# JohnVithor/RL-Rust

Measured on AMD Instinct MI355X. Metric: env-steps/sec, FrozenLake-8x8 Q-learning, 2^20 envs, 1/2/4/8 GPUs, higher is better.
Workload: dtype f64 TD arithmetic; shared Q int64 fixed point 2^-40 (range proven, |Q| <= 2048, no clamp)

## Files before the change

### rl-rust_amd/csrc/rl_device.h

```cpp
#pragma once
#include <hip/hip_runtime.h>
#include <stdint.h>

#include "rl_kparams.h"
#include "rl_taxi.h"

#pragma clang fp contract(off)

namespace rlamd {

constexpr double MIN_POSITIVE = 2.2250738585072014e-308;

__device__ __forceinline__ uint32_t xor3(uint32_t a, uint32_t b, uint32_t c) {
    uint32_t r;
    asm("v_bitop3_b32 %0, %1, %2, %3 bitop3:0x96" : "=v"(r) : "v"(a), "v"(b), "v"(c));
    return r;
}
struct Rng {
    uint32_t s0, s1, s2, s3;
    __device__ __forceinline__ void advance() {
        const uint32_t t = s1 << 9;
        const uint32_t n1 = xor3(s1, s2, s0), n2 = xor3(s2, s0, t), n0 = xor3(s0, s3, s1), n3 = s3 ^ s1;
        s0 = n0; s1 = n1; s2 = n2;
        s3 = __builtin_rotateleft32(n3, 11);
// ... 251 lines not shown
        y = t - (e - x);
        y = add_exponent(y, k);
    } else {
        t = with_hi(0.0, (uint32_t)((0x3ff - k) << 20));
        y = x - (e + t);
        y += 1.0;
        y = add_exponent(y, k);
    }
    return y;
}

__device__ inline double rl_tanh(double x) {
    const double tiny = 1.0e-300;
    double t, z;
    const int32_t jx = (int32_t)hi_word(x);
    const int32_t ix = jx & 0x7fffffff;
    if (ix >= 0x7ff00000) {
        if (jx >= 0) return 1.0 / x + 1.0;
        return 1.0 / x - 1.0;
    }
    if (ix < 0x40360000) {
        if (ix < 0x3c800000) return x * (1.0 + x);
        if (ix >= 0x3ff00000) {
            t = rl_expm1(2.0 * __builtin_fabs(x));
            z = 1.0 - 2.0 / (t + 2.0);
        } else {
            t = rl_expm1(-2.0 * __builtin_fabs(x));
            z = -t / (t + 2.0);
        }
    } else {
        z = 1.0 - tiny;
    }
    return jx >= 0 ? z : -z;
}

__device__ __forceinline__ double max_rs(double a, double b) { return (a > b || b != b) ? a : b; }
__device__ __forceinline__ double min_rs(double a, double b) { return (a < b || b != b) ? a : b; }
__device__ __forceinline__ double sigmoid_(double v) { return 1.0 / (1.0 + rl_exp(-v)); }
template <int ACT>
__device__ __forceinline__ double act_t(double v) {
    if constexpr (ACT == RL_ACT_TANH) return rl_tanh(v);
    else if constexpr (ACT == RL_ACT_RELU) return max_rs(v, 0.0);
    else if constexpr (ACT == RL_ACT_LEAKY_RELU) return max_rs(v, 0.1 * v);
    else if constexpr (ACT == RL_ACT_RELU6) return min_rs(max_rs(v, 0.0), 6.0);
    else if constexpr (ACT == RL_ACT_LEAKY_RELU6) return __builtin_fmin(__builtin_fmax(v, 0.1 * v), 6.0);
    else if constexpr (ACT == RL_ACT_SIGMOID) return sigmoid_(v);
    else if constexpr (ACT == RL_ACT_SWISH) return v * sigmoid_(v);
    else if constexpr (ACT == RL_ACT_HARD_SWISH) return (v * min_rs(max_rs(v + 3.0, 0.0), 6.0)) / 6.0;
    else return v;
}
template <int ACT>
__device__ __forceinline__ double act_pt(double v) {
    if constexpr (ACT == RL_ACT_TANH) { const double t = rl_tanh(v); return 1.0 - t * t; }
    else if constexpr (ACT == RL_ACT_RELU) return v > 0.0 ? 1.0 : 0.0;
    else if constexpr (ACT == RL_ACT_LEAKY_RELU) return v > 0.0 ? 1.0 : 0.01;
    else if constexpr (ACT == RL_ACT_RELU6) return (v > 0.0 && v < 6.0) ? 1.0 : 0.0;
    else if constexpr (ACT == RL_ACT_LEAKY_RELU6) return (v > 0.0 && v < 6.0) ? 1.0 : 0.01;
    else if constexpr (ACT == RL_ACT_SIGMOID) { const double sg = sigmoid_(v); return sg * (1.0 - sg); }
    else if constexpr (ACT == RL_ACT_SWISH) { const double e = rl_exp(v); return (e * (v + e + 1.0)) / ((e + 1.0) * (e + 1.0)); }
    else if constexpr (ACT == RL_ACT_HARD_SWISH) return v > -3.0 ? (2.0 * v + 3.0) / 6.0 : 0.0;
    else return 1.0;
}
__device__ inline double act_f(int act, double v) {
    switch (act) {
    case RL_ACT_TANH: return act_t<RL_ACT_TANH>(v);
    case RL_ACT_RELU: return act_t<RL_ACT_RELU>(v);
    case RL_ACT_LEAKY_RELU: return act_t<RL_ACT_LEAKY_RELU>(v);
    case RL_ACT_RELU6: return act_t<RL_ACT_RELU6>(v);
    case RL_ACT_LEAKY_RELU6: return act_t<RL_ACT_LEAKY_RELU6>(v);
    case RL_ACT_SIGMOID: return act_t<RL_ACT_SIGMOID>(v);
    case RL_ACT_SWISH: return act_t<RL_ACT_SWISH>(v);
    case RL_ACT_HARD_SWISH: return act_t<RL_ACT_HARD_SWISH>(v);
    default: return v;
    }
}
__device__ inline double act_fp(int act, double v) {
    switch (act) {
    case RL_ACT_TANH: return act_pt<RL_ACT_TANH>(v);
    case RL_ACT_RELU: return act_pt<RL_ACT_RELU>(v);
    case RL_ACT_LEAKY_RELU: return act_pt<RL_ACT_LEAKY_RELU>(v);
    case RL_ACT_RELU6: return act_pt<RL_ACT_RELU6>(v);
    case RL_ACT_LEAKY_RELU6: return act_pt<RL_ACT_LEAKY_RELU6>(v);
    case RL_ACT_SIGMOID: return act_pt<RL_ACT_SIGMOID>(v);
    case RL_ACT_SWISH: return act_pt<RL_ACT_SWISH>(v);
    case RL_ACT_HARD_SWISH: return act_pt<RL_ACT_HARD_SWISH>(v);
    default: return 1.0;
    }
}

__device__ __forceinline__ double ucb_value(double q, double c, double lnt, double n) {
    return q + c * __builtin_sqrt(lnt / (n + MIN_POSITIVE));
}

template <int A>
__device__ __forceinline__ uint32_t ucb_known(const double (&v)[A], const uint64_t (&n)[A], double c, double lnt,
                                              double (&u)[A]) {
    const double b0 = c * __builtin_sqrt(lnt * 0x1p1022);
    const bool c_fin = __builtin_fabs(c) < 0x1p1020;
    uint32_t need = 0;
#pragma unroll
    for (int i = 0; i < A; ++i) {
        const bool z = n[i] == 0ull, nf = !__builtin_isfinite(v[i]) && c_fin;
        u[i] = z ? v[i] + b0 : (nf ? v[i] : 0.0);
        need |= (!z && !nf) ? (1u << i) : 0u;
    }
    return need;
}
template <int A>
__device__ __forceinline__ void ucb_fill(const double (&v)[A], const uint64_t (&n)[A], double c, double lnt,
                                         uint32_t need, double (&u)[A]) {
#pragma unroll
    for (int i = 0; i < A; ++i)
        if ((need >> i) & 1u) u[i] = ucb_value(v[i], c, lnt, (double)n[i]);
}

constexpr uint64_t QNAN_BITS = 0x7FF8000000000000ull;
__device__ __forceinline__ double as_f64(uint64_t u) { return __longlong_as_double((long long)u); }
__device__ __forceinline__ uint64_t f64_bits(double x) { return (uint64_t)__double_as_longlong(x); }
__device__ __forceinline__ double canon_nan(double x) { return x != x ? as_f64(QNAN_BITS) : x; }
__device__ __forceinline__ uint32_t f64_code(double x) {
    return ((uint32_t)((uint64_t)__double_as_longlong(x) >> 52)) & 0x7ffu;
}
__device__ __forceinline__ int fq_grid(uint32_t code) { return (int)(code > 1u ? code : 1u) - 1075; }
__device__ __forceinline__ uint32_t nf_flag(double x) { return x != x ? QF_NAN : (x > 0.0 ? QF_PINF : QF_NINF); }
__device__ __forceinline__ double nf_value(uint32_t f) {
    if ((f & QF_NAN) || ((f & QF_PINF) && (f & QF_NINF))) return as_f64(QNAN_BITS);
    return (f & QF_PINF) ? __builtin_inf() : -__builtin_inf();
}
__device__ __forceinline__ int64_t fq_raw(double d, int e) {
    return (int64_t)__builtin_rint(__builtin_ldexp(d, -e));
}
template <int A>
__device__ __forceinline__ uint32_t argmax_max_f64(const double (&v)[A], double &m) {
    m = v[0];
    uint32_t r = 0;
#pragma unroll
    for (int i = 1; i < A; ++i) {
        const bool gt = v[i] > m;
        m = gt ? v[i] : m;
        r = gt ? (uint32_t)i : r;
    }
    return r;
}

constexpr int64_t Q_RAW_MAX = (int64_t)1 << 51;

__device__ __forceinline__ int64_t rint_i64_small(double x) {
    const double y = x + 0x1.8p52;
    return (int64_t)((uint64_t)__double_as_longlong(y) - 0x4338000000000000ull);
}
__device__ __forceinline__ int64_t q_fix_inrange(double d) { return rint_i64_small(d * 0x1p40); }
__device__ __forceinline__ double q_val(int64_t raw) {
    return __longlong_as_double((long long)(0x40B8000000000000ull + (uint64_t)raw)) - 6144.0;
}
template <int A>
__device__ __forceinline__ uint32_t argmax_i64(const int64_t (&v)[A]) {
    int64_t m = v[0];
    uint32_t r = 0;
#pragma unroll
    for (int i = 1; i < A; ++i)
        if (v[i] > m) { m = v[i]; r = (uint32_t)i; }
    return r;
}
template <int A>
__device__ __forceinline__ int64_t max_i64(const int64_t (&v)[A]) {
    int64_t m = v[0];
#pragma unroll
    for (int i = 1; i < A; ++i) m = v[i] > m ? v[i] : m;
    return m;
}
template <class T>
__device__ __forceinline__ T opq(T x) {
    asm("" : "+v"(x));
    return x;
}
template <int A, class T>
__device__ __forceinline__ T pick(const T (&v)[A], uint32_t i) {
    T r = opq(v[0]);
#pragma unroll
    for (int j = 1; j < A; ++j) r = (i == (uint32_t)j) ? opq(v[j]) : r;
    return r;
}

template <int A>
__device__ __forceinline__ uint32_t argmax(const double (&v)[A]) {
    double m = v[0];
    uint32_t r = 0;
#pragma unroll
    for (int i = 1; i < A; ++i)
        if (v[i] > m) { m = v[i]; r = (uint32_t)i; }
    return r;
}
template <int A>
__device__ __forceinline__ double vmax(const double (&v)[A]) {
    double m = v[0];
#pragma unroll
    for (int i = 1; i < A; ++i)
        if (v[i] > m) m = v[i];
    return m;
}
__device__ __forceinline__ uint32_t cdf_search(const double *cdf, uint32_t n, double u) {
    uint32_t lo = 0, hi = n;
    while (lo < hi) {
        const uint32_t mid = (lo + hi) >> 1;
        if (cdf[mid] > u) hi = mid; else lo = mid + 1;
    }
    return lo < n ? lo : 0u;
}

struct EnvTables {
    const uint32_t *trans;
    const double *cdf;
    uint32_t n_start, max_steps;
    double th1, th2, th3, trunc_reward;
    int32_t fixed_start;
    int32_t slippery;
    uint32_t S;
};
template <bool AM, int A>
__device__ __forceinline__ uint32_t tidx(const EnvTables &t, uint32_t s, uint32_t a) {
    return AM ? a * t.S + s : s * (uint32_t)A + a;
}
__device__ __forceinline__ uint32_t start_state(const EnvTables &t, double u) {
    return t.fixed_start >= 0 ? (uint32_t)t.fixed_start : cdf_search(t.cdf, t.n_start, u);
}

__device__ __forceinline__ uint32_t start_list_search(const EnvTables &t, double u) {
    const uint32_t *cells = (const uint32_t *)(t.cdf + t.n_start);
    uint32_t c = 0;
    bool found = false;
    for (uint32_t j = 0; j < t.n_start; ++j) {
        const bool hit = !found && t.cdf[j] > u;
        c = hit ? cells[j] : c;
        found = found || hit;
    }
    return c;
}

template <int ENV> struct EnvDev;

template <bool EDITED, int SLIP, bool AM, bool MAPS = false>
__device__ __forceinline__ void fl_advance(bool doR, bool doS, uint32_t &pos, uint32_t &z, uint32_t w, Rng &r,
                                           const EnvTables &t, uint32_t &s2, double &rew, bool &term) {
    const bool trunc = doS && z >= t.max_steps;
    const bool st = doS && !trunc;
    uint32_t i = 0, s0 = 0;
    if constexpr (MAPS) {
        const bool slip = SLIP == 1 || (SLIP < 0 && t.slippery);
        const bool drawn = t.fixed_start < 0;
        s0 = drawn ? 0u : (uint32_t)t.fixed_start;
        if ((slip && st) || (drawn && doR)) {
            const double u = uniform01(r);
            const uint32_t iu = (t.th1 > u) ? 0u : (t.th2 > u) ? 1u : (t.th3 > u) ? 2u : 0u;
            i = (st && (w & (1u << 24))) ? iu : 0u;
            if (drawn) {
                const uint32_t c = start_list_search(t, u);
                s0 = doR ? c : 0u;
            }
        }
    } else if (SLIP == 1 || (SLIP < 0 && t.slippery)) {
        if (st) {
            const double u = uniform01(r);
            if (w & (1u << 24)) i = (t.th1 > u) ? 0u : (t.th2 > u) ? 1u : (t.th3 > u) ? 2u : 0u;
        }
    }
    const uint32_t o = (w >> (8 * i)) & 0xffu;
    const double r_bit = EDITED ? 10.0 : 1.0, r_else = EDITED ? -1.0 : 0.0;
    s2 = st ? (o & 63u) : ((EDITED && trunc) ? pos : (MAPS && doR ? s0 : 0u));
    rew = st ? ((o & 64u) ? r_bit : r_else) : ((EDITED && trunc) ? -1.0 : 0.0);
    term = trunc || (st && (o & 128u) != 0u);
    z = doR ? 0u : (st ? z + 1u : z);
    pos = s2;
}

template <> struct EnvDev<RL_ENV_FROZEN_LAKE> {
    static constexpr int A = 4;
    __device__ static __forceinline__ uint32_t reset(uint32_t &z, Rng &, const EnvTables &) {
        z = 0;
        return 0u;
    }
    template <int SLIP = -1, bool AM = false>
    __device__ static __forceinline__ void step(uint32_t &pos, uint32_t &z, uint32_t a, Rng &r,
                                                const EnvTables &t, uint32_t &s2, double &rew,
                                                bool &term) {
        if (z >= t.max_steps) { s2 = 0; rew = 0.0; term = true; return; }
        z += 1;
        const uint32_t w = t.trans[tidx<AM, 4>(t, pos, a)];
        uint32_t i = 0;
        if (SLIP == 1 || (SLIP < 0 && t.slippery)) {
            const double u = uniform01(r);
            if (w & (1u << 24)) i = (t.th1 > u) ? 0u : (t.th2 > u) ? 1u : (t.th3 > u) ? 2u : 0u;
        }
        const uint32_t o = (w >> (8 * i)) & 0xffu;
        s2 = o & 63u;
        rew = (o & 64u) ? 1.0 : 0.0;
        term = (o & 128u) != 0;
        pos = s2;
    }
};

template <> struct EnvDev<RL_ENV_FROZEN_LAKE_EDITED> {
    static constexpr int A = 4;
    __device__ static __forceinline__ uint32_t reset(uint32_t &z, Rng &, const EnvTables &) {
        z = 0;
        return 0u;
    }
// ... 263 lines not shown
```

### rl-rust_amd/csrc/rl_train_impl.h

```cpp
#pragma once
#include <type_traits>

#include "rl_device.h"
#include "rl_net.h"

namespace rlamd {

constexpr uint32_t POOL_ITEM_BYTES = 10u;
struct SmemLayout {
    uint32_t st, misc, q, sum, cnt, sfl, qf, n, nd, t, list, rcp, tr, cdf, lrec, trc, qd, rm, total;
    uint32_t trc_cap;
    uint32_t nrcp;
};
__host__ __device__ inline uint32_t align16(uint32_t x) { return (x + 15u) & ~15u; }

constexpr uint32_t BJ_LDS_STATES = 22u * 11u * 2u;
__host__ __device__ inline bool bj_compact(int env, int ucb) { return env == RL_ENV_BLACKJACK && !ucb; }
__host__ __device__ inline bool bj_nonterminal(uint32_t s) {
    const uint32_t p = s >> 6, d = (s >> 1) & 31u;
    return p <= 21u && d <= 10u;
}
__host__ __device__ inline uint32_t bj_row(uint32_t s) {
    const uint32_t p = s >> 6, r = s & 63u;
    return (p * 11u + (r >> 1)) * 2u + (r & 1u);
// ... 180 lines not shown
    e.pad[0] = e.pad[1] = e.pad[2] = 0;
    e.reward = L.epi_reward;
    p.elog[(uint64_t)(c % p.elog_cap) * p.L + lane] = e;
    p.elog_cnt[lane] = c + 1u;
}

__device__ __forceinline__ void write_record(const KParams &p, uint32_t k, uint64_t lane, uint32_t kind,
                                             uint32_t s, uint32_t a, uint32_t s2, uint32_t a2, double r,
                                             bool term, double td, uint32_t mode) {
    rl_step_record rec;
    rec.s = s;
    rec.s2 = s2;
    rec.a = (uint8_t)a;
    rec.a2 = (uint8_t)a2;
    rec.term = (uint8_t)term;
    rec.mode = (uint8_t)mode;
    rec.kind = (uint8_t)kind;
    rec.pad[0] = rec.pad[1] = rec.pad[2] = 0;
    rec.r = r;
    rec.td = td;
    p.rec[(uint64_t)k * p.L + lane] = rec;
}

template <int A>
__device__ __forceinline__ void trace_visit(const KParams &p, uint64_t lane, uint32_t s, uint32_t a,
                                            uint32_t &cnt) {
    const uint64_t Ls = p.L;
    uint32_t j = p.slot_of[(uint64_t)s * Ls + lane];
    if (j < cnt && p.tlist[(uint64_t)j * Ls + lane] == s) {
        double *e = &p.trace[((uint64_t)j * A + a) * Ls + lane];
        *e = *e + 1.0;
    } else {
        j = cnt++;
        p.tlist[(uint64_t)j * Ls + lane] = (uint16_t)s;
        p.slot_of[(uint64_t)s * Ls + lane] = (uint16_t)j;
#pragma unroll
        for (int b = 0; b < A; ++b) p.trace[((uint64_t)j * A + b) * Ls + lane] = (uint32_t)b == a ? 1.0 : 0.0;
    }
}

template <int A, class RowFn, class Fn>
__device__ __forceinline__ void trace_sweep(const KParams &p, uint64_t lane, uint32_t nv, RowFn &&row_fn, Fn &&fn) {
    constexpr uint32_t TC = 4;
    const uint64_t Ls = p.L;
    for (uint32_t j0 = 0; j0 < nv; j0 += TC) {
        uint32_t o[TC];
        double ev[TC][A];
#pragma unroll
        for (uint32_t c = 0; c < TC; ++c) {
            const bool in = j0 + c < nv;
            const uint32_t j = in ? j0 + c : j0;
            o[c] = p.tlist[(uint64_t)j * Ls + lane];
#pragma unroll
            for (int b = 0; b < A; ++b) ev[c][b] = p.trace[((uint64_t)j * A + b) * Ls + lane];
        }
#pragma unroll
        for (uint32_t c = 0; c < TC; ++c) {
            if (j0 + c < nv) {
                const uint32_t j = j0 + c;
                row_fn(o[c]);
#pragma unroll
                for (int b = 0; b < A; ++b) {
                    fn(o[c], (uint32_t)b, ev[c][b]);
                    p.trace[((uint64_t)j * A + b) * Ls + lane] = ev[c][b] * p.gl;
                }
            }
        }
    }
}

constexpr uint32_t SWEEP_U = 4;
__device__ __forceinline__ uint64_t pslot(const KParams &p, uint32_t j, uint64_t lane) {
    return lane * (uint64_t)(p.S * p.A) + j;
}
struct PairCache {
    uint16_t *TRI;
    double *TRE;
    uint32_t cap, nthr, tid;
    __device__ __forceinline__ uint32_t ixi_t(uint32_t j, uint32_t t) const { return j * (nthr + 2u) + t; }
    __device__ __forceinline__ uint32_t ixe_t(uint32_t j, uint32_t t) const { return j * (nthr + 1u) + t; }
    __device__ __forceinline__ uint32_t ixi(uint32_t j) const { return ixi_t(j, tid); }
    __device__ __forceinline__ uint32_t ixe(uint32_t j) const { return ixe_t(j, tid); }
};
template <int A>
__device__ __forceinline__ void pair_visit(const KParams &p, const PairCache &c, uint64_t lane, uint32_t s,
                                           uint32_t a, uint32_t &np) {
    const uint64_t Ls = p.L;
    const uint32_t id = s * (uint32_t)A + a, id0 = s * (uint32_t)A;
    const uint32_t nl = np < c.cap ? np : c.cap;
    uint32_t hit = 0xffffffffu;
    bool same_state = false;
    constexpr uint32_t TB = 8;
    for (uint32_t j0 = 0; j0 < nl; j0 += TB) {
        uint32_t w[TB];
#pragma unroll
        for (uint32_t k = 0; k < TB; ++k) w[k] = c.TRI[c.ixi(j0 + k < nl ? j0 + k : j0)] & 0x7fffu;
#pragma unroll
        for (uint32_t k = 0; k < TB; ++k) {
            if (j0 + k < nl) {
                if (w[k] == id) hit = j0 + k;
                if (w[k] - id0 < (uint32_t)A) same_state = true;
            }
        }
    }
    if (hit != 0xffffffffu) {
        c.TRE[c.ixe(hit)] += 1.0;
        return;
    }
    if (np > c.cap) {
        const uint32_t j = p.slot_of[(uint64_t)id * Ls + lane];
        if (j >= c.cap && j < np && (p.tlist[pslot(p, j, lane)] & 0x7fffu) == id) {
            double *e = &p.trace[pslot(p, j, lane)];
            *e = *e + 1.0;
            return;
        }
    }
    const uint32_t j = np++;
    if (j < c.cap) {
        c.TRI[c.ixi(j)] = (uint16_t)(id | (same_state ? 0u : 0x8000u));
        c.TRE[c.ixe(j)] = 1.0;
    } else {
        uint32_t *vw = &p.vbits[(uint64_t)(s >> 5) * Ls + lane];
        const uint32_t vb = *vw, bit = 1u << (s & 31u);
        const bool first = !same_state && (vb & bit) == 0u;
        if ((vb & bit) == 0u) *vw = vb | bit;
        p.tlist[pslot(p, j, lane)] = (uint16_t)(id | (first ? 0x8000u : 0u));
        p.slot_of[(uint64_t)id * Ls + lane] = (uint16_t)j;
        p.trace[pslot(p, j, lane)] = 1.0;
    }
}
__device__ __forceinline__ void pair_clear(const KParams &p, const PairCache &c, uint64_t lane, uint32_t np) {
    if (np <= c.cap) return;
    const uint32_t nw = (p.S + 31u) >> 5;
    for (uint32_t w = 0; w < nw; ++w) p.vbits[(uint64_t)w * p.L + lane] = 0u;
}
__device__ __forceinline__ void pair_cache_load(const KParams &p, const PairCache &c, uint64_t lane, uint32_t np) {
    const uint32_t nl = np < c.cap ? np : c.cap;
    for (uint32_t j = 0; j < nl; ++j) {
        c.TRI[c.ixi(j)] = p.tlist[pslot(p, j, lane)];
        c.TRE[c.ixe(j)] = p.trace[pslot(p, j, lane)];
    }
}
__device__ __forceinline__ void pair_cache_store(const KParams &p, const PairCache &c, uint64_t lane, uint32_t np) {
    const uint32_t nl = np < c.cap ? np : c.cap;
    for (uint32_t j = 0; j < nl; ++j) {
        p.tlist[pslot(p, j, lane)] = c.TRI[c.ixi(j)];
        p.trace[pslot(p, j, lane)] = c.TRE[c.ixe(j)];
    }
}

constexpr uint32_t QF_MASK = QF_NAN | QF_PINF | QF_NINF, QF_PENDING = 4u;
__device__ __forceinline__ uint32_t value_flags(double q) { return __builtin_isfinite(q) ? 0u : nf_flag(q); }

template <int AGENT, int POLICY, int SEL, int ALGO>
constexpr bool fix_possible() {
    return AGENT == RL_AGENT_ONE_STEP && POLICY == RL_POLICY_TABULAR &&
           !(SEL == RL_SEL_UCB && ALGO == RL_ALGO_EXPECTED_SARSA);
}

constexpr uint32_t CARVE_OWN = 0xffffffffu;
template <int ENV, int AGENT, int POLICY, int SEL, int ALGO, bool INSTR, bool FQ, int SLIP = -1, int SWEEP = -1,
          bool PACK = false, int RS = -1, int EPI = -1, bool POP = false>
__device__ __forceinline__ void train_shared_body(const KParams &p, unsigned long long *pop_row = nullptr,
                                                  uint32_t carve_n_start = CARVE_OWN) {
    using E = EnvDev<ENV>;
    constexpr int A = E::A;
    constexpr int P = POLICY == RL_POLICY_DOUBLE ? 2 : 1;
    constexpr bool UCB = SEL == RL_SEL_UCB;
    constexpr bool TRACES = AGENT == RL_AGENT_TRACES;
    constexpr bool SPEC = UCB && ALGO == RL_ALGO_EXPECTED_SARSA;
    static_assert(FQ || fix_possible<AGENT, POLICY, SEL, ALGO>(), "no range proof: f64 only");
    constexpr bool BJC = ENV == RL_ENV_BLACKJACK && !UCB;
    const uint32_t S = p.S, SA = S * (uint32_t)A, PSA = (uint32_t)P * SA;
    const uint32_t SL = BJC ? BJ_LDS_STATES : S, SAL = SL * (uint32_t)A, PSAL = (uint32_t)P * SAL;

    extern __shared__ __attribute__((aligned(16))) unsigned char smem[];
    const uint32_t tid = threadIdx.x, nthr = blockDim.x;
    constexpr bool PAIRS = TRACES && !SPEC;
    constexpr bool QSH = qsh_layout(FQ ? 1 : 0, UCB ? 1 : 0, P, ALGO);
    uint32_t carve_ns = p.n_start;
    if constexpr (POP) carve_ns = carve_n_start == CARVE_OWN ? p.n_start : carve_n_start;
    const SmemLayout lay = smem_layout(ENV, P, UCB ? (SPEC ? 2 : 1) : 0, TRACES ? (PAIRS ? 2 : 1) : 0, S, A, carve_ns,
                                       nthr, p.trc_kb, FQ ? 1 : 0, p.ucb_pack, QSH ? 1 : 0);
    unsigned long long *Q = (unsigned long long *)(smem + lay.q);
    double *QD = (double *)(smem + lay.qd);
    double2 *RM = (double2 *)(smem + lay.rm);
    unsigned long long *SUM = (unsigned long long *)(smem + lay.sum);
    uint32_t *CNT = (uint32_t *)(smem + lay.cnt);
    uint16_t *CNT16 = (uint16_t *)(smem + lay.cnt);
    uint32_t *W = (uint32_t *)(smem + lay.cnt);
    uint32_t *SFLW = (uint32_t *)(smem + (SPEC ? lay.qf : lay.sfl));
    uint8_t *SFL8 = (uint8_t *)(smem + (SPEC ? lay.qf : lay.sfl));
    constexpr uint32_t SFL_SH = SPEC ? QF_PENDING : 0u;
    uint32_t *QF = (uint32_t *)(smem + lay.qf);
    uint8_t *QF8 = (uint8_t *)(smem + lay.qf);
    unsigned long long *N = (unsigned long long *)(smem + lay.n);
    unsigned long long *T = (unsigned long long *)(smem + lay.t);
    uint32_t *NL = (uint32_t *)(smem + lay.n);
    uint32_t *D32 = (uint32_t *)(smem + lay.nd);
    uint16_t *D16 = (uint16_t *)(smem + lay.nd);
    uint16_t *LIST = (uint16_t *)(smem + lay.list);
    uint32_t *LISTN = (uint32_t *)(smem + lay.list + align16(PSAL * 2u));
    uint32_t *TR = (uint32_t *)(smem + lay.tr);
    double *RCP = (double *)(smem + lay.rcp);
    uint32_t *GCODE = (uint32_t *)(smem + lay.misc);

    unsigned long long *ACC = (unsigned long long *)(smem + lay.st);
    constexpr bool LDS_AM = false;
    auto lrow = [&](uint32_t s) -> uint32_t {
        if constexpr (BJC) return bj_row(s);
        else return s;
    };
    auto qi = [&](uint32_t tbl, uint32_t s, uint32_t a) -> uint32_t {
        return LDS_AM ? tbl * SAL + a * SL + lrow(s) : tbl * SAL + lrow(s) * (uint32_t)A + a;
    };
    auto dense_of = [&](uint32_t j) -> uint32_t {
        if constexpr (!LDS_AM && !BJC) return j;
        const uint32_t tbl = j / SAL, r = j - tbl * SAL;
        const uint32_t row = LDS_AM ? r % SL : r / (uint32_t)A, a = LDS_AM ? r / SL : r % (uint32_t)A;
        const uint32_t s = BJC ? bj_dense(row) : row;
        return tbl * SA + s * (uint32_t)A + a;
    };
    auto lds_of = [&](uint32_t i) -> uint32_t {
        if constexpr (!LDS_AM) return i;
        const uint32_t tbl = i / SA, r = i - tbl * SA;
        return qi(tbl, r / (uint32_t)A, r % (uint32_t)A);
    };
    if (tid < STATS_W) ACC[tid] = 0ull;
    if (tid == 0) GCODE[0] = 0u;
    for (uint32_t i = tid; i < lay.nrcp; i += nthr) RCP[i] = i == 0 ? 0.0 : 1.0 / (double)i;
    for (uint32_t j = tid; j < PSAL; j += nthr) {
        Q[j] = (unsigned long long)p.q_base[dense_of(j)];
        SUM[j] = 0ull;
        if constexpr (QSH) QD[j] = q_val((int64_t)Q[j]);
    }
    if constexpr (FQ && !TRACES) {
        for (uint32_t j = tid; j < PSAL; j += nthr) W[j] = 0u;
    } else {
        for (uint32_t i = tid; i < (PSAL + 1u) / 2u; i += nthr) CNT[i] = 0u;
    }
    if constexpr (FQ && TRACES && !SPEC)
        for (uint32_t i = tid; i < (PSAL + 3u) / 4u; i += nthr) SFLW[i] = 0u;
    if constexpr (TRACES) { if (tid == 0) LISTN[0] = 0u; }
    if constexpr (UCB) {
        if constexpr (SPEC) {
            for (uint32_t j = tid; j < PSAL; j += nthr) QF8[j] = (uint8_t)value_flags(as_f64(Q[j]));
            for (uint32_t i = tid; i < SA; i += nthr) NL[i] = 0u;
            if (!p.ucb_pack)
                for (uint32_t i = tid; i < (SA + 1u) / 2u; i += nthr) D32[i] = 0u;
        } else {
            for (uint32_t i = tid; i < SA; i += nthr) N[lds_of(i)] = (unsigned long long)p.n_base[i];
        }
        if (tid == 0) {
            T[0] = p.t_base[0]; T[1] = 0ull;
            if constexpr (SPEC) *(uint32_t *)(T + 2) = 0u;
        }
    }
    if constexpr (env_wide(ENV)) {
        for (uint32_t i = tid; i < SA; i += nthr) ((uint16_t *)TR)[lds_of(i)] = ((const uint16_t *)p.trans)[i];
    } else if constexpr (ENV != RL_ENV_TAXI && ENV != RL_ENV_BLACKJACK) {
        for (uint32_t i = tid; i < SA; i += nthr) TR[lds_of(i)] = p.trans[i];
    }
    if constexpr (env_map_start(ENV))
        for (uint32_t i = tid; i < p.n_start * 3u; i += nthr)
            ((uint32_t *)(smem + lay.cdf))[i] = ((const uint32_t *)p.start_cdf)[i];
    const bool sweep = SWEEP == 1 || PSAL <= nthr;
    const bool rmx = QSH && A == 4 && sweep;
    if (rmx) {
        for (uint32_t r = tid; r < SL; r += nthr) {
            double v[A], m;
#pragma unroll
            for (int i = 0; i < A; ++i) v[i] = q_val(p.q_base[r * (uint32_t)A + i]);
            const uint32_t a = argmax_max_f64<A>(v, m);
            RM[r] = make_double2(m, as_f64((uint64_t)a));
        }
    }
    __syncthreads();

    EnvTables tabs;
    tabs.trans = TR; tabs.cdf = p.start_cdf; tabs.n_start = p.n_start; tabs.max_steps = p.max_steps;
    if constexpr (env_map_start(ENV)) tabs.cdf = (const double *)(smem + lay.cdf);
    tabs.th1 = p.th1; tabs.th2 = p.th2; tabs.th3 = p.th3; tabs.trunc_reward = p.trunc_reward;
    tabs.fixed_start = p.fixed_start;
    tabs.slippery = p.slippery;
    tabs.S = S;

    const uint32_t gl = (tid >> 6) * p.lpw + (tid & 63u);
    const uint64_t lane = (uint64_t)blockIdx.x * p.G + gl;
    const bool active = (tid & 63u) < p.lpw && gl < p.G && lane < p.L;
    LaneRegs L;
    lane_load(p, lane, active, L);
    uint32_t tcnt = 0, trace_states = 0;
    constexpr bool ESU = UCB && ALGO == RL_ALGO_EXPECTED_SARSA;
    double lnt_es = 0.0;
    bool lnt_ok = false;
    auto lnt_cur = [&](unsigned long long t) -> double {
        if (!lnt_ok) { lnt_es = rl_log((double)t); lnt_ok = true; }
        return lnt_es;
    };
    auto ucount = [&](uint32_t s, uint32_t i, bool with_step) -> uint64_t {
        const uint32_t idx = qi(0u, s, i);
        if constexpr (SPEC) {
            if (p.ucb_pack) {
                const uint32_t w = NL[idx];
                return p.n_base[s * (uint32_t)A + i] + (uint64_t)(w >> 16) + (with_step ? (uint64_t)(w & 0xffffu) : 0ull);
            }
            return p.n_base[s * (uint32_t)A + i] + (uint64_t)NL[idx] + (with_step ? (uint64_t)D16[idx] : 0ull);
        } else {
            return N[idx];
        }
    };
    if constexpr (TRACES) tcnt = active ? p.tcnt[lane] : 0u;
    const PairCache pc{(uint16_t *)(smem + lay.trc), (double *)(smem + lay.trc + align16(lay.trc_cap * (nthr + 2u) * 2u)),
                       lay.trc_cap, nthr, tid};
    constexpr int PBW = ENV == RL_ENV_CLIFF_WALKING ? 6 : 8;
    constexpr bool POOL = PAIRS && pair_pool_env(ENV);
    static_assert(!POOL || A == 4, "a state's pair bits sit in one bitmap word");
    const uint32_t pw = tid >> 6, plid = tid & 63u;
    const uint64_t plane0 = (uint64_t)blockIdx.x * p.G + (uint64_t)pw * p.lpw;
    const bool pwave = (uint64_t)pw * p.lpw < p.G && plane0 < p.L;
    uint16_t *const PT = (uint16_t *)(smem + lay.trc) + pw * lay.trc_cap;
    double *const PE = (double *)(smem + lay.trc + align16(lay.trc_cap * (nthr >> 6) * 2u)) + pw * lay.trc_cap;
    uint4 *const LR = (uint4 *)(smem + lay.lrec) + pw * 64u;
    uint16_t *const HT = p.tlist + plane0 * SA;
    double *const HE = p.trace + plane0 * SA;
    auto pool_tag = [&](uint32_t q) -> uint32_t { return PT[q]; };
    auto pool_get = [&](uint32_t q, uint32_t &tg, double &e) {
        tg = PT[q];
        e = PE[q];
    };
    auto pool_put = [&](uint32_t q, uint32_t tg, double e) {
        PT[q] = (uint16_t)tg;
        PE[q] = e;
    };
    uint32_t npool = 0;
    uint32_t pbits[PBW];
#pragma unroll
    for (int i = 0; i < PBW; ++i) pbits[i] = 0u;
    auto pbits_word = [&](uint32_t wi) -> uint32_t {
        uint32_t w = opq(pbits[0]);
#pragma unroll
        for (int i = 1; i < PBW; ++i) w = wi == (uint32_t)i ? opq(pbits[i]) : w;
        return w;
    };
    auto pbits_set = [&](uint32_t id) {
#pragma unroll
        for (int i = 0; i < PBW; ++i) pbits[i] |= (id >> 5) == (uint32_t)i ? (1u << (id & 31u)) : 0u;
    };
    if constexpr (PAIRS && !POOL) { if (active) pair_cache_load(p, pc, lane, tcnt); }
    if constexpr (POOL) {
        npool = pwave ? p.tcnt[plane0] : 0u;
        const uint32_t nl = npool < lay.trc_cap ? npool : lay.trc_cap;
        for (uint32_t q = plid; q < nl; q += 64u) pool_put(q, HT[q], HE[q]);
        __syncthreads();
        constexpr uint32_t TB = 8;
        for (uint32_t q0 = 0; q0 < nl; q0 += TB) {
            uint32_t t[TB];
#pragma unroll
            for (uint32_t k = 0; k < TB; ++k) t[k] = pool_tag(q0 + k < nl ? q0 + k : q0);
#pragma unroll
            for (uint32_t k = 0; k < TB; ++k)
                if (q0 + k < nl && ((t[k] >> 8) & 63u) == plid) pbits_set(t[k] & 0xffu);
        }
        for (uint32_t q0 = nl; q0 < npool; q0 += TB) {
            uint32_t t[TB];
#pragma unroll
            for (uint32_t k = 0; k < TB; ++k) t[k] = HT[q0 + k < npool ? q0 + k : q0];
#pragma unroll
            for (uint32_t k = 0; k < TB; ++k)
                if (q0 + k < npool && ((t[k] >> 8) & 63u) == plid) pbits_set(t[k] & 0xffu);
        }
    }

    constexpr uint64_t row_mask = 0x0707070707070707ull >> (8 * (8 - A));
    auto row_flags = [&](uint32_t tbl, uint32_t s) -> uint64_t {
        static_assert(A <= 6, "flag rows span at most two LDS words");
        const uint32_t off = qi(tbl, s, 0u), w = off >> 2;
        const uint64_t two = (uint64_t)QF[w] | ((uint64_t)QF[w + 1u] << 32);
        return (two >> ((off & 3u) * 8u)) & row_mask;
    };
    auto flag_nan = [](uint32_t f) -> bool { return (f & QF_NAN) || (f & (QF_PINF | QF_NINF)) == (QF_PINF | QF_NINF); };
    auto val = [&](int64_t raw) -> double {
        if constexpr (FQ) return as_f64((uint64_t)raw);
        else return q_val(raw);
    };
    auto qd_row = [&](uint32_t s, double (&v)[A]) {
        if constexpr (A == 4) {
// ... 43 lines not shown
                for (int i = 0; i < A; ++i) v[i] = P == 2 ? (as_f64(ra[i]) + as_f64(rb[i])) / 2.0 : as_f64(ra[i]);
                return argmax<A>(v);
            } else {
                return argmax_i64<A>(ra);
            }
        } else {
            double u[A], v[A];
            uint64_t n[A];
            const double lnt = ESU ? lnt_cur(T[0]) : rl_log((double)T[0]);
#pragma unroll
            for (int i = 0; i < A; ++i) {
                v[i] = val(ra[i]);
                if constexpr (P == 2) v[i] = (v[i] + val(rb[i])) / 2.0;
                n[i] = ucount(s, (uint32_t)i, false);
            }
            uint32_t need = ucb_known<A>(v, n, p.ucb_c, lnt, u);
            const bool c_fin = __builtin_fabs(p.ucb_c) < 0x1p1020;
            bool decided = (need & 1u) == 0u && u[0] != u[0];
#pragma unroll
            for (int i = 0; i < A; ++i)
                decided = decided || (c_fin && ((need >> i) & 1u) == 0u && u[i] == __builtin_inf());
            if (need && !decided) ucb_fill<A>(v, n, p.ucb_c, lnt, need, u);
            return argmax<A>(u);
        }
    };
    auto select_lazy = [&](uint32_t s) -> uint32_t {
        bool explore = L.eps != 0.0;
        if (explore) explore = eps_test(L.rng, L.eps);
        if (explore) return uniform_action<A>(L.rng);
        int64_t ra[A], rb[A];
        load_rows(s, ra, rb);
        if constexpr (FQ) {
            double v[A];
#pragma unroll
            for (int i = 0; i < A; ++i) v[i] = P == 2 ? (as_f64(ra[i]) + as_f64(rb[i])) / 2.0 : as_f64(ra[i]);
            return argmax<A>(v);
        } else {
            return argmax_i64<A>(ra);
        }
    };
    constexpr bool PACKC = PACK && !FQ;
    auto contribute = [&](uint32_t idx, int64_t sum, uint32_t n) -> bool {
        if constexpr (PACKC) {
            const unsigned long long v = (unsigned long long)(sum * 2048) + n;
            if (sweep) { atomicAdd(&SUM[idx], v); return false; }
            return (atomicAdd(&SUM[idx], v) & 2047ull) == 0ull;
        }
        const uint32_t sh = (idx & 1u) * 16u;
        bool first = false;
        if (sweep) atomicAdd(&CNT[idx >> 1], n << sh);
        else first = ((atomicAdd(&CNT[idx >> 1], n << sh) >> sh) & 0xffffu) == 0u;
        if (sum) atomicAdd(&SUM[idx], (unsigned long long)sum);
        return first;
    };
    auto settle = [&](uint32_t idx) -> double {
        const int64_t packed = (int64_t)SUM[idx];
        const unsigned long long qold = Q[idx];
        const uint32_t n = PACKC ? (uint32_t)(packed & 2047) : (uint32_t)CNT16[idx];
        const int64_t sum = PACKC ? (packed >> 11) : packed;
        const double rc = (sweep || n < lay.nrcp) ? RCP[n] : 1.0 / (double)n;
        const double sd = PACKC ? __longlong_as_double((long long)(0x4338000000000000ull + (uint64_t)sum)) - 0x1.8p52
                                : (double)sum;
        const double y = __builtin_trunc(sd * rc) + 0x1.8p52;
        const int64_t md = (int64_t)((uint64_t)__double_as_longlong(y) - 0x4338000000000000ull);
        const unsigned long long q = qold + (unsigned long long)md;
        Q[idx] = q;
        const double v = q_val((int64_t)q);
        if constexpr (QSH) QD[idx] = v;
        SUM[idx] = 0ull;
        if constexpr (!PACKC) CNT16[idx] = 0;
        return v;
    };
    auto settle_quad = [&](uint32_t t) {
        double m = settle(t);
        uint32_t a = t & 3u;
        auto combine = [&](auto dpp_ctrl_tag, uint32_t bit) {
            constexpr int C = decltype(dpp_ctrl_tag)::value;
            const uint64_t mb = f64_bits(m);
            const uint32_t pl = (uint32_t)__builtin_amdgcn_mov_dpp((int)(uint32_t)mb, C, 0xF, 0xF, false);
            const uint32_t ph = (uint32_t)__builtin_amdgcn_mov_dpp((int)(uint32_t)(mb >> 32), C, 0xF, 0xF, false);
            const uint32_t pa = (uint32_t)__builtin_amdgcn_mov_dpp((int)a, C, 0xF, 0xF, false);
            const double pm = as_f64(((uint64_t)ph << 32) | pl);
            const bool mine_lo = (t & bit) == 0u;
            const double lo = mine_lo ? m : pm, hi = mine_lo ? pm : m;
            const uint32_t la = mine_lo ? a : pa, ha = mine_lo ? pa : a;
            const bool up = hi > lo;
            m = up ? hi : lo;
            a = up ? ha : la;
        };
        combine(std::integral_constant<int, 0xB1>{}, 1u);
        combine(std::integral_constant<int, 0x4E>{}, 2u);
        if ((t & 3u) == 0u) RM[t >> 2] = make_double2(m, as_f64((uint64_t)a));
    };
    auto settle_fq = [&](uint32_t idx) {
        const uint32_t w = W[idx], n = w & 0xfffu;
        const uint32_t f = w >> 28;
        if (n == 0u && f == 0u) return;
        double dl;
        if (f) {
            dl = nf_value(f);
        } else {
            const double rc = (sweep || n < lay.nrcp) ? RCP[n] : 1.0 / (double)n;
            dl = __builtin_ldexp((double)(int64_t)SUM[idx] * rc, fq_grid(((w >> 16) & 0xfffu) - 1u));
        }
        const double q = canon_nan(as_f64(Q[idx]) + dl);
        Q[idx] = f64_bits(q);
        SUM[idx] = 0ull;
        W[idx] = 0u;
        if constexpr (SPEC) QF8[idx] = (uint8_t)value_flags(q);
    };
    uint32_t *const CNTR = CNT;
    const bool rsweep = POOL || (uint32_t)P * SL <= nthr;
    auto qi_row = [&](uint32_t tbl, uint32_t row, uint32_t a) -> uint32_t {
        return LDS_AM ? tbl * SAL + a * SL + row : tbl * SAL + row * (uint32_t)A + a;
    };
    auto contrib_tr = [&](uint32_t idx, double d, int e) {
        if (__builtin_isfinite(d)) {
            const double y = __builtin_ldexp(d, -e) + 0x1.8p52;
            const int64_t raw = (int64_t)((uint64_t)__double_as_longlong(y) - 0x4338000000000000ull);
            if (raw) atomicAdd(&SUM[idx], (unsigned long long)raw);
        } else {
            atomicOr(&SFLW[idx >> 2], (nf_flag(d) << SFL_SH) << ((idx & 3u) * 8u));
        }
    };
    auto settle_row = [&](uint32_t rid, int e) {
        const uint32_t n = CNTR[rid];
        if (n == 0u) return;
        const double rc = n < lay.nrcp ? RCP[n] : 1.0 / (double)n;
        const uint32_t tbl = rid / SL, row = rid - tbl * SL;
#pragma unroll
        for (int b = 0; b < A; ++b) {
            const uint32_t idx = qi_row(tbl, row, (uint32_t)b);
            const uint32_t f = ((uint32_t)SFL8[idx] >> SFL_SH) & QF_MASK;
            const double dl = f ? nf_value(f) : __builtin_ldexp((double)(int64_t)SUM[idx] * rc, e);
            const double q = canon_nan(as_f64(Q[idx]) + dl);
            Q[idx] = f64_bits(q);
            SUM[idx] = 0ull;
            if constexpr (SPEC) QF8[idx] = (uint8_t)value_flags(q);
            else if (f) SFL8[idx] = 0;
        }
        CNTR[rid] = 0u;
    };
    uint32_t c_train = 0, c_eval = 0, c_tep = 0, c_eep = 0;
    unsigned long long *const RSUM = &ACC[4];
    constexpr bool LANE_CNT = ENV == RL_ENV_FROZEN_LAKE && AGENT == RL_AGENT_ONE_STEP &&
                              POLICY == RL_POLICY_TABULAR && !UCB && !FQ;
    uint32_t n_train = 0;
    const uint32_t train_ep0 = L.train_ep;

    constexpr bool TXPF = ENV == RL_ENV_TAXI && (UCB || RS == 0);
    uint32_t wtx = 0;
    if constexpr (TXPF) wtx = p.trans[(L.s < S ? L.s : 0u) * (uint32_t)A + (L.a < (uint32_t)A ? L.a : 0u)];
    const bool rs_on = (!UCB && RS != 0) && (RS == 1 || p.reset_step);
    for (uint32_t k = 0; k < p.K; ++k) {
        const bool alive = L.mode != RL_MODE_DONE;
        bool doR = alive && L.need_reset;
        bool doS = alive && !L.need_reset;
        const uint32_t mode_before = L.mode;
        uint32_t s2 = 0, a2 = 0;
        double r = 0.0;
        bool term = false;
        int64_t ra2[A], rb2[A];
        bool fused = false;
        if constexpr (!UCB && RS != 0) {
            if (RS == 1 || p.reset_step) {
                if (doR && !FUSE_MAX) {
                    const uint32_t s0 = E::reset(L.z, L.rng, tabs);
                    L.ready = true;
                    L.a = select_lazy(s0);
                    L.s = s0;
                    L.need_reset = false;
                    L.epi_reward = 0.0;
                    L.epi_len = 0;
                    fused = true;
                } else if (doR) {
                    const uint32_t s0 = E::reset(L.z, L.rng, tabs);
                    L.ready = true;
                    load_rows(s0, ra2, rb2);
                    int32_t pre = -1;
                    if constexpr (FUSE_MAX) {
                        if constexpr (FQ) {
                            double v[A], m;
#pragma unroll
                            for (int i = 0; i < A; ++i) v[i] = as_f64(ra2[i]);
                            pre = (int32_t)argmax_max_f64<A>(v, m);
                        } else if (rmx) {
                            pre = (int32_t)(uint32_t)f64_bits(RM[s0].y);
                        } else {
                            double v[A], m;
                            qd_row(s0, v);
                            pre = (int32_t)argmax_max_f64<A>(v, m);
                        }
                    }
                    L.a = select(s0, ra2, rb2, pre);
                    L.s = s0;
                    L.need_reset = false;
                    L.epi_reward = 0.0;
                    L.epi_len = 0;
                    fused = true;
                }
                doR = false;
                doS = alive;
            }
        }
        if constexpr (env_wide(ENV)) {
            uint32_t pos = L.s;
            fl_advance_wide<env_fl_edited(ENV), SLIP, LDS_AM>(doR, doS, pos, L.z, L.a, L.rng, tabs, s2, r, term);
            L.ready = doR ? true : (term ? false : L.ready);
        } else if constexpr (env_fl_family(ENV)) {
            uint32_t pos = L.s;
            const uint32_t w = tabs.trans[tidx<LDS_AM, 4>(tabs, L.s, L.a)];
            fl_advance<env_fl_edited(ENV), SLIP, LDS_AM, env_map_start(ENV)>(doR, doS, pos, L.z, w, L.rng, tabs, s2,
                                                                             r, term);
            L.ready = doR ? true : (term ? false : L.ready);
        } else if (doR) {
            s2 = E::reset(L.z, L.rng, tabs);
            L.ready = true;
        } else if (doS) {
            uint32_t pos = L.s;
            if constexpr (TXPF) E::step_word(L.z, wtx, tabs, s2, r, term);
            else E::template step<SLIP, LDS_AM>(pos, L.z, L.a, L.rng, tabs, s2, r, term);
            if (term) L.ready = false;
        }
        if (k > 0 && !rs_on) __syncthreads();
        bool sel_nan0 = false, tgt_nf = false;
        if constexpr (SPEC) {
            const uint64_t f0 = row_flags(0u, s2), f1 = P == 2 ? row_flags(1u, s2) : 0ull;
            sel_nan0 = flag_nan((uint32_t)f0 & 0xffu) || (P == 2 && flag_nan((uint32_t)f1 & 0xffu));
            tgt_nf = ((((P == 2 && !L.dflag) ? f1 : f0) & row_mask) != 0ull);
        }
        const bool train_lane = doS && L.mode == RL_MODE_TRAIN;
        if (!SPEC || !(sel_nan0 && (tgt_nf || !train_lane))) load_rows(s2, ra2, rb2);
        else {
#pragma unroll
            for (int i = 0; i < A; ++i) ra2[i] = rb2[i] = 0;
        }
        int64_t qa_raw_pre = 0;
        constexpr bool QAE2 = TRACES && !SPEC;
        if constexpr (QAE2) {
            if (BJC && !bj_nonterminal(L.s)) qa_raw_pre = 0;
            else qa_raw_pre = (int64_t)Q[qi((P == 2 && !L.dflag) ? 1u : 0u, L.s, L.a)];
        }
        uint32_t rm_pad = 0;
        double qa_pre = 0.0;
        double rmaxd = 0.0;
        int32_t rarg = -1;
        if constexpr (FUSE_MAX) {
            if constexpr (FQ) {
                double v[A];
#pragma unroll
                for (int i = 0; i < A; ++i) v[i] = as_f64(ra2[i]);
                rarg = (int32_t)argmax_max_f64<A>(v, rmaxd);
                asm volatile("" : "+v"(rarg), "+v"(rmaxd));
            } else {
                if (rmx) {
                    const double2 rm = RM[s2];
                    rmaxd = rm.x;
                    rarg = (int32_t)(uint32_t)f64_bits(rm.y);
                    rm_pad = (uint32_t)(f64_bits(rm.y) >> 32);
                    if (!rs_on) qa_pre = QD[qi(0u, L.s, L.a)];
                } else {
                    double v[A];
                    if (BJC && !bj_nonterminal(s2)) {
#pragma unroll
                        for (int i = 0; i < A; ++i) v[i] = q_val(ra2[i]);
                    } else {
                        qd_row(s2, v);
                    }
                    rarg = (int32_t)argmax_max_f64<A>(v, rmaxd);
                    asm volatile("" : "+v"(rarg), "+v"(rmaxd));
                }
            }
        }
        if (alive) a2 = sel_nan0 ? 0u : select(s2, ra2, rb2, rarg);
        if constexpr (TXPF) wtx = p.trans[s2 * (uint32_t)A + a2];
        uint32_t d_own = 0xffffffffu;
        if constexpr (SPEC) {
            if (alive) {
                const uint32_t idx = qi(0, s2, a2);
                if (p.ucb_pack) {
                    if ((atomicAdd(&NL[idx], 1u) & 0xffffu) == 0u) d_own = idx;
                } else {
                    const uint32_t sh = (idx & 1u) * 16u;
                    if (((atomicAdd(&D32[idx >> 1], 1u << sh) >> sh) & 0xffffu) == 0u) d_own = idx;
                }
            }
            const uint32_t c = (uint32_t)__popcll(__ballot(alive));
            if ((tid & 63u) == 0 && c) atomicAdd(&T[1], (unsigned long long)c);
            uint32_t *ARR = (uint32_t *)(T + 2);
            __threadfence_block();
            if ((tid & 63u) == 0) atomicAdd(ARR, 1u);
            if (__ballot(train_lane && !tgt_nf)) {
                const uint32_t goal = (k + 1u) * (nthr >> 6);
                while (__builtin_amdgcn_readfirstlane(__hip_atomic_load(ARR, __ATOMIC_RELAXED,
                                                                        __HIP_MEMORY_SCOPE_WORKGROUP)) < goal)
                    __builtin_amdgcn_s_sleep(1);
                __threadfence_block();
            }
            lnt_ok = false;
        } else if constexpr (UCB) {
            __syncthreads();
            if (alive) atomicAdd(&N[qi(0, s2, a2)], 1ull);
            const uint32_t c = (uint32_t)__popcll(__ballot(alive));
            if ((tid & 63u) == 0 && c) atomicAdd(&T[0], (unsigned long long)c);
        }
        const bool train = doS && L.mode == RL_MODE_TRAIN;
// ... 1036 lines not shown
```

Before: 360.3 billion.

## Add entry-owned TD update path for FrozenLake Q-learning with per-state row max

Adds a specialised training loop for deterministic FrozenLake Q-learning in which each thread owns one Q entry. Envs atomically count visits per entry (separately for terminal-by-step-limit transitions), and the owner then applies a single mean TD update computed from counts times a per-entry TD code. The owner also recomputes the row max/argmax via DPP quad reductions into a double-buffered row-max table, so envs read argmax directly. This replaces per-env atomic Q updates with counting plus one owner update per step, relying on all transitions from an entry being identical (non-slippery) and adding a barrier each step.

Result: slower. 328.6 billion (-8.8%).

```diff
diff --git a/rl-rust_amd/csrc/rl_device.h b/rl-rust_amd/csrc/rl_device.h
--- a/rl-rust_amd/csrc/rl_device.h
+++ b/rl-rust_amd/csrc/rl_device.h
@@ -427,6 +427,15 @@
 __device__ __forceinline__ int64_t q_fix_inrange(double d) { return rint_i64_small(d * 0x1p40); }
 __device__ __forceinline__ double q_val(int64_t raw) {
     return __longlong_as_double((long long)(0x40B8000000000000ull + (uint64_t)raw)) - 6144.0;
+}
+__host__ __device__ inline double entry_td_code(double lr40, double gamma, double r, double fq, double qa) {
+    const double td = r + gamma * fq - qa;
+    return (lr40 * td + 0x1.8p52) - 0x1.8p52;
+}
+__host__ __device__ inline int64_t entry_td_mean(double c1, uint32_t n1, double c2, uint32_t n2, double rcp) {
+    const double sd = c1 * (double)n1 + c2 * (double)n2;
+    const double y = __builtin_trunc(sd * rcp) + 0x1.8p52;
+    return (int64_t)(__builtin_bit_cast(uint64_t, y) - 0x4338000000000000ull);
 }
 template <int A>
 __device__ __forceinline__ uint32_t argmax_i64(const int64_t (&v)[A]) {
diff --git a/rl-rust_amd/csrc/rl_train_impl.h b/rl-rust_amd/csrc/rl_train_impl.h
--- a/rl-rust_amd/csrc/rl_train_impl.h
+++ b/rl-rust_amd/csrc/rl_train_impl.h
@@ -356,6 +356,25 @@
 constexpr uint32_t QF_MASK = QF_NAN | QF_PINF | QF_NINF, QF_PENDING = 4u;
 __device__ __forceinline__ uint32_t value_flags(double q) { return __builtin_isfinite(q) ? 0u : nf_flag(q); }
 
+__device__ __forceinline__ void quad_max_arg(uint32_t t, double &m, uint32_t &a) {
+    auto combine = [&](auto dpp_ctrl_tag, uint32_t bit) {
+        constexpr int C = decltype(dpp_ctrl_tag)::value;
+        const uint64_t mb = f64_bits(m);
+        const uint32_t pl = (uint32_t)__builtin_amdgcn_mov_dpp((int)(uint32_t)mb, C, 0xF, 0xF, false);
+        const uint32_t ph = (uint32_t)__builtin_amdgcn_mov_dpp((int)(uint32_t)(mb >> 32), C, 0xF, 0xF, false);
+        const uint32_t pa = (uint32_t)__builtin_amdgcn_mov_dpp((int)a, C, 0xF, 0xF, false);
+        const double pm = as_f64(((uint64_t)ph << 32) | pl);
+        const bool mine_lo = (t & bit) == 0u;
+        const double lo = mine_lo ? m : pm, hi = mine_lo ? pm : m;
+        const uint32_t la = mine_lo ? a : pa, ha = mine_lo ? pa : a;
+        const bool up = hi > lo;
+        m = up ? hi : lo;
+        a = up ? ha : la;
+    };
+    combine(std::integral_constant<int, 0xB1>{}, 1u);
+    combine(std::integral_constant<int, 0x4E>{}, 2u);
+}
+
 template <int AGENT, int POLICY, int SEL, int ALGO>
 constexpr bool fix_possible() {
     return AGENT == RL_AGENT_ONE_STEP && POLICY == RL_POLICY_TABULAR &&
@@ -382,6 +401,10 @@
     const uint32_t tid = threadIdx.x, nthr = blockDim.x;
     constexpr bool PAIRS = TRACES && !SPEC;
     constexpr bool QSH = qsh_layout(FQ ? 1 : 0, UCB ? 1 : 0, P, ALGO);
+    constexpr bool ENTRY_TD = ENV == RL_ENV_FROZEN_LAKE && AGENT == RL_AGENT_ONE_STEP &&
+                              POLICY == RL_POLICY_TABULAR && SEL == RL_SEL_EPS_GREEDY &&
+                              ALGO == RL_ALGO_QLEARNING && !FQ && PACK && SLIP == 0 && SWEEP == 1 && RS == 0 &&
+                              !INSTR && !POP;
     uint32_t carve_ns = p.n_start;
     if constexpr (POP) carve_ns = carve_n_start == CARVE_OWN ? p.n_start : carve_n_start;
     const SmemLayout lay = smem_layout(ENV, P, UCB ? (SPEC ? 2 : 1) : 0, TRACES ? (PAIRS ? 2 : 1) : 0, S, A, carve_ns,
@@ -436,7 +459,7 @@
     for (uint32_t j = tid; j < PSAL; j += nthr) {
         Q[j] = (unsigned long long)p.q_base[dense_of(j)];
         SUM[j] = 0ull;
-        if constexpr (QSH) QD[j] = q_val((int64_t)Q[j]);
+        if constexpr (QSH && !ENTRY_TD) QD[j] = q_val((int64_t)Q[j]);
     }
     if constexpr (FQ && !TRACES) {
         for (uint32_t j = tid; j < PSAL; j += nthr) W[j] = 0u;
@@ -786,6 +809,96 @@
     uint32_t wtx = 0;
     if constexpr (TXPF) wtx = p.trans[(L.s < S ? L.s : 0u) * (uint32_t)A + (L.a < (uint32_t)A ? L.a : 0u)];
     const bool rs_on = (!UCB && RS != 0) && (RS == 1 || p.reset_step);
+    if constexpr (ENTRY_TD) {
+        uint32_t *const CN = (uint32_t *)SUM;
+        double2 *const RM1 = (double2 *)QD;
+        uint32_t ent = qi(0u, L.s, L.a);
+        auto count_in = [&](uint32_t par) {
+            if (L.mode == RL_MODE_TRAIN && !L.need_reset)
+                atomicAdd(&CN[par * PSAL + ent], L.z >= tabs.max_steps ? 0x10000u : 1u);
+        };
+        if (p.K) count_in(0u);
+        auto run = [&](auto own_tag) {
+            constexpr bool OWN = decltype(own_tag)::value;
+            const uint32_t wo = OWN ? TR[tid] : 0u;
+            const uint32_t so = wo & 63u;
+            const double ro = (wo & 64u) ? 1.0 : 0.0;
+            unsigned long long qo = OWN ? Q[tid] : 0ull;
+            double qv = q_val((int64_t)qo);
+            for (uint32_t k = 0; k < p.K; ++k) {
+                const bool alive = L.mode != RL_MODE_DONE;
+                const bool doR = alive && L.need_reset, doS = alive && !L.need_reset;
+                uint32_t s2 = 0, a2 = 0;
+                double r = 0.0;
+                bool term = false;
+                uint32_t pos = L.s;
+                const uint32_t w = tabs.trans[ent];
+                fl_advance<false, SLIP, LDS_AM, false>(doR, doS, pos, L.z, w, L.rng, tabs, s2, r, term);
+                L.ready = doR ? true : (term ? false : L.ready);
+                __syncthreads();
+                const uint32_t par = k & 1u;
+                const double2 *const RMk = par ? RM1 : RM;
+                double2 *const RMn = par ? RM : RM1;
+                uint32_t cw = 0;
+                double m1 = 0.0;
+                if constexpr (OWN) {
+                    cw = CN[par * PSAL + tid];
+                    m1 = RMk[so].x;
+                }
+                const uint32_t rarg = ((const uint32_t *)(RMk + s2))[2];
+                if (alive) {
+                    bool explore = L.eps != 0.0;
+                    if (explore) explore = eps_test(L.rng, L.eps);
+                    a2 = explore ? uniform_action<A>(L.rng) : rarg;
+                }
+                double rc = 0.0;
+                if constexpr (OWN) rc = RCP[(cw & 0xffffu) + (cw >> 16)];
+                const bool train = doS && L.mode == RL_MODE_TRAIN;
+                bool tr = false, ev = false;
+                if (doS) {
+                    if (train) {
+                        const double nw = L.eps * p.eps_dm - p.eps_ds;
+                        L.eps = (term && !(p.eps_final > nw)) ? nw : L.eps;
+                    }
+                    after_step<EPI>(p, L, s2, a2, r, term, tr, ev);
+                    if (tr) atomicAdd(RSUM, (unsigned long long)rint_i64_small(L.epi_reward * 65536.0));
+                } else if (doR) {
+                    L.s = s2;
+                    L.a = a2;
+                    L.need_reset = false;
+                    L.epi_reward = 0.0;
+                    L.epi_len = 0;
+                }
+                ent = qi(0u, L.s, L.a);
+                n_train += train ? 1u : 0u;
+                if (EPI > 0 || (EPI < 0 && p.episodic)) {
+                    c_eval += (uint32_t)__popcll(__ballot(doS && !train));
+                    c_eep += (uint32_t)__popcll(__ballot(ev));
+                }
+                if (k + 1u < p.K) count_in(par ^ 1u);
+                if constexpr (OWN) {
+                    if (__ballot(cw != 0u)) {
+                        const uint32_t n1 = cw & 0xffffu, n2 = cw >> 16;
+                        const double c1 = entry_td_code(p.lr40, p.gamma, ro, m1, qv);
+                        double c2 = 0.0;
+                        if (n2) c2 = entry_td_code(p.lr40, p.gamma, 0.0, RMk[0].x, qv);
+                        qo += (unsigned long long)entry_td_mean(c1, n1, c2, n2, rc);
+                        qv = q_val((int64_t)qo);
+                        CN[par * PSAL + tid] = 0u;
+                        double m = qv;
+                        uint32_t am = tid & 3u;
+                        quad_max_arg(tid, m, am);
+                        if ((tid & 3u) == 0u) RMn[tid >> 2] = make_double2(m, as_f64((uint64_t)am));
+                    } else if ((tid & 3u) == 0u) {
+                        RMn[tid >> 2] = RMk[tid >> 2];
+                    }
+                }
+            }
+            if constexpr (OWN) Q[tid] = qo;
+        };
+        if ((uint32_t)__builtin_amdgcn_readfirstlane((int)tid) < PSAL) run(std::true_type{});
+        else run(std::false_type{});
+    } else
     for (uint32_t k = 0; k < p.K; ++k) {
         const bool alive = L.mode != RL_MODE_DONE;
         bool doR = alive && L.need_reset;
```
